# superxslam/SuperOdom

Measured on AMD Instinct MI355X. Metric: icp_registrations_per_sec, higher is better.
Workload: dtype f64

## Files before the change

superodom_amd/build.py:

```python
import os
import subprocess
import sys

HERE = os.path.dirname(os.path.abspath(__file__))
CSRC = os.path.join(HERE, "csrc")
LIBDIR = os.path.join(HERE, "lib")
LIB = os.path.join(LIBDIR, "libsoicp.so")
SOURCES = ["kernels.hip", "map_kernels.hip", "icp_context.cpp", "staging.cpp", "sequence.cpp", "batch.cpp", "localization.cpp", "prefilter.cpp", "cloud_steps.cpp", "multi_gpu.cpp",
           "local_map.cpp", "device_map.cpp", "localization_sequence.cpp", "feature_kernels.hip", "feature_extraction.cpp", "corr_kernels.hip", "corr_sums_kernels.hip", "corr_geometry_kernels.hip", "correspondences.cpp", "pose_prior.cpp"]
HEADERS = ["kernels.h", "device_idioms.h", "map_kernels.h", "device_map.h", "lm_solver.h", "local_map.h", "so_math.h", "deskew_math.h", "untimed_math.h", "plane_fit.h", "plane_factor.h", "ctx.h", "reg_plan.h", "feature_kernels.h", "corr_kernels.h", "pose_prior.h", "eval_kernel_body.inc", "solve_kernel_body.inc", os.path.join("..", "..", "include", "so_icp.h")]
ARCH = "gfx950"
COMMON = ["-O3", "-std=c++17", "-fPIC", "-ffp-contract=off", "-Wall", "-Wno-unused-function", "-Wno-unused-result"]
COMMON += os.environ.get("SOICP_EXTRA_CXXFLAGS", "").split()


def _stale():
    if not os.path.exists(LIB):
        return True
    t = os.path.getmtime(LIB)
    deps = [os.path.join(CSRC, s) for s in SOURCES + HEADERS] + [os.path.abspath(__file__)]
    return any(os.path.getmtime(d) > t for d in deps if os.path.exists(d))


def build(force=False, verbose=False):
    if not force and not _stale():
        return LIB
    hipcc = os.environ.get("HIPCC", "/opt/rocm/bin/hipcc")
    os.makedirs(LIBDIR, exist_ok=True)
    objs = []
    for s in SOURCES:
        o = os.path.join(LIBDIR, os.path.splitext(s)[0] + ".o")
        lang = ["-x", "hip"] if s.endswith(".hip") else []
        cmd = [hipcc, f"--offload-arch={ARCH}"] + lang + ["-c", os.path.join(CSRC, s), "-o", o] + COMMON
        if verbose:
            print(" ".join(cmd))
        subprocess.check_call(cmd)
        objs.append(o)
    cmd = [hipcc, f"--offload-arch={ARCH}", "-shared", "-o", LIB] + objs + ["-ldl"]
    if verbose:
        print(" ".join(cmd))
    subprocess.check_call(cmd)
    return LIB


if __name__ == "__main__":
    print(build(force="--force" in sys.argv, verbose=True))
```

superodom_amd/csrc/kernels.h:

```cpp
#pragma once
#include <hip/hip_runtime_api.h>

#include <cstddef>
#include <cstdint>

#include "lm_solver.h"
#include "pose_prior.h"
#include "so_math.h"

namespace soicp {

struct DevMapView {
  const float4* pts;
  const uint32_t* cell_start;
  const int32_t* cube_slot;
  int32_t nc;
  uint32_t ncell1;
  double inv_cell;
  int32_t origin[3];
  uint32_t n_points;
  uint32_t n_slots;
};

struct RegBeginArgs { double pose[7]; int32_t max_outer, lm_max; uint32_t chain_expect, pad; };

struct MatchParams {
  float plane_res;
  float sq_max_dist_f;
  double max_point_dist;
  int32_t ablate;
  unsigned long long* kdbg;
  uint32_t* packed_leftover;
  int32_t pack_light;
  int32_t skip_near_pass;
  uint32_t chunk_cap;
  uint32_t chain_expect;
  struct DevState* hring[2];
  unsigned long long seq_base;
  int32_t publish_prev;
  int32_t begin, begin_max_surface_features;
  uint32_t begin_n;
  RegBeginArgs begin_args;
  const unsigned long long* begin_ctr;
  struct DevState* begin_state;
};

struct EvalParams {
  double a2;
  int32_t variant;
  int32_t ablate;
  uint32_t n_queries, q_stride;
  struct DevState* hring[2];
  unsigned long long seq_base;
  int32_t defer_publish;
  uint32_t chain_expect;
  int32_t chain_next;
  double chain_delta[7];
  unsigned long long epoch_base;
  void* peer_inbox[8];
  int32_t peer_rank, peer_world;
  unsigned long long timeout_ticks;
// ... 132 lines not shown
```

superodom_amd/csrc/kernels.hip:

```cpp
#include <hip/hip_runtime.h>
#include <hip/hip_ext.h>

#include <cstddef>
#include <cstdlib>
#include <cstring>
#include <type_traits>

#ifdef SO_LM_STAMPS
#define SO_LM_STAMP(dbg, i) do { if (dbg) (dbg)[i] = wall_clock64(); } while (0)
#endif
#include "device_idioms.h"
#include "kernels.h"
#include "plane_factor.h"
#include "plane_fit.h"
#include "pose_prior.h"

namespace soicp {

#define SO_MATCH_SUCCESS 0
#define SO_MATCH_NOT_ENOUGH 1
#define SO_MATCH_TOO_FAR 2
#define SO_MATCH_BAD_PCA 3
#define SO_MATCH_INVALID 4
#define SO_MATCH_MSE 5
// ... 304 lines not shown

__device__ __forceinline__ int32_t imed3(int32_t a, int32_t b, int32_t c) {
  int32_t r;
  asm("v_med3_i32 %0, %1, %2, %3" : "=v"(r) : "v"(a), "v"(b), "v"(c));
  return r;
}

constexpr int32_t kKeyEmpty = 0x7FFFFFFF;

struct Net8 {
  int32_t a0, a1, a2, a3, a4, a5, a6, a7;
  __device__ __forceinline__ void init() { a0 = a1 = a2 = a3 = a4 = a5 = a6 = a7 = kKeyEmpty; }
  __device__ __forceinline__ void push(int32_t k) {
    a7 = imed3(a6, a7, k);
    a6 = imed3(a5, a6, k);
    a5 = imed3(a4, a5, k);
    a4 = imed3(a3, a4, k);
    a3 = imed3(a2, a3, k);
    a2 = imed3(a1, a2, k);
    a1 = imed3(a0, a1, k);
    a0 = a0 < k ? a0 : k;
  }
};

constexpr float kApproxAbsErr = 2e-5f;
typedef float float2v __attribute__((ext_vector_type(2)));
__device__ __forceinline__ float2v approx_d2_pair(float2v m2qx, float2v m2qy, float2v m2qz, float2v qq, float2v cx, float2v cy,
                                                  float2v cz, float2v cc) {
  float2v v = cc + qq;
  v = __builtin_elementwise_fma(m2qx, cx, v);
  v = __builtin_elementwise_fma(m2qy, cy, v);
  v = __builtin_elementwise_fma(m2qz, cz, v);
  return v;
}
__device__ __forceinline__ int32_t make_key(float d2a, uint32_t jloc_uniform, uint32_t keep_mask) {
  int32_t r;
  asm("v_bfi_b32 %0, %1, %2, %3" : "=v"(r) : "v"(keep_mask), "v"(d2a), "s"(jloc_uniform));
  return r;
}
__device__ __forceinline__ int32_t make_key_v(float d2a, uint32_t jloc, uint32_t keep_mask) {
  int32_t r;
  asm("v_bfi_b32 %0, %1, %2, %3" : "=v"(r) : "v"(keep_mask), "v"(d2a), "v"(jloc));
  return r;
}
__device__ __forceinline__ int32_t approx_key(float m2qx, float m2qy, float m2qz, float qq, float cx, float cy, float cz,
                                              float cc, uint32_t jloc, uint32_t keep_mask) {
  float v = cc + qq;
  v = __builtin_fmaf(m2qx, cx, v);
  v = __builtin_fmaf(m2qy, cy, v);
  v = __builtin_fmaf(m2qz, cz, v);
  return (int32_t)((__float_as_uint(v) & keep_mask) | (jloc & ~keep_mask));
}

__device__ __forceinline__ void publish_state_to(DevState* dst, const DevState* st, unsigned long long seq, int tid, int nthreads);

#ifndef SO_KNN_FILTER
#define SO_KNN_FILTER 1
#endif
__device__ __forceinline__ float wave_min_f32(float v) {
  const int inf = 0x7F800000;
#define SO_DPP_MIN(ctrl, rows) v = fminf(v, __int_as_float(__builtin_amdgcn_update_dpp(inf, __float_as_int(v), ctrl, rows, 0xF, false)))
  SO_DPP_MIN(0x111, 0xF); SO_DPP_MIN(0x112, 0xF); SO_DPP_MIN(0x114, 0xF); SO_DPP_MIN(0x118, 0xF);
  SO_DPP_MIN(0x142, 0xA); SO_DPP_MIN(0x143, 0xC);
#undef SO_DPP_MIN
  return __int_as_float(__builtin_amdgcn_readlane(__float_as_int(v), 63));
}

__device__ __forceinline__ int row_min_i32(int v) {
  v = min(v, __builtin_amdgcn_update_dpp(v, v, 0x121, 0xF, 0xF, false)); v = min(v, __builtin_amdgcn_update_dpp(v, v, 0x122, 0xF, 0xF, false));
  v = min(v, __builtin_amdgcn_update_dpp(v, v, 0x124, 0xF, 0xF, false)); v = min(v, __builtin_amdgcn_update_dpp(v, v, 0x128, 0xF, 0xF, false));
  return v;
}
__device__ __forceinline__ int row_max_i32(int v) {
  v = max(v, __builtin_amdgcn_update_dpp(v, v, 0x121, 0xF, 0xF, false)); v = max(v, __builtin_amdgcn_update_dpp(v, v, 0x122, 0xF, 0xF, false));
  v = max(v, __builtin_amdgcn_update_dpp(v, v, 0x124, 0xF, 0xF, false)); v = max(v, __builtin_amdgcn_update_dpp(v, v, 0x128, 0xF, 0xF, false));
  return v;
}
__device__ __forceinline__ float row_min_f32(float v) {
#define SO_ROR_F(ctrl) __int_as_float(__builtin_amdgcn_update_dpp(__float_as_int(v), __float_as_int(v), ctrl, 0xF, 0xF, false))
  v = fminf(v, SO_ROR_F(0x121)); v = fminf(v, SO_ROR_F(0x122)); v = fminf(v, SO_ROR_F(0x124)); v = fminf(v, SO_ROR_F(0x128));
#undef SO_ROR_F
  return v;
}
__device__ __forceinline__ unsigned long long wave_min_u64(unsigned long long v) {
#pragma unroll
  for (int off = 32; off > 0; off >>= 1) {
    const unsigned long long o = __shfl_xor(v, off, 64);
    v = o < v ? o : v;
  }
  return v;
}
__device__ __forceinline__ uint32_t row_inclusive_scan_u32(uint32_t v) {
  v += (uint32_t)__builtin_amdgcn_update_dpp(0, (int)v, 0x111, 0xF, 0xF, true);
  v += (uint32_t)__builtin_amdgcn_update_dpp(0, (int)v, 0x112, 0xF, 0xF, true);
  v += (uint32_t)__builtin_amdgcn_update_dpp(0, (int)v, 0x114, 0xF, 0xF, true);
  v += (uint32_t)__builtin_amdgcn_update_dpp(0, (int)v, 0x118, 0xF, 0xF, true);
  return v;
}
__device__ __forceinline__ uint32_t max_over_rows(uint32_t v) {
  return max(max((uint32_t)__builtin_amdgcn_readlane((int)v, 0), (uint32_t)__builtin_amdgcn_readlane((int)v, 16)),
             max((uint32_t)__builtin_amdgcn_readlane((int)v, 32), (uint32_t)__builtin_amdgcn_readlane((int)v, 48)));
}
__device__ __forceinline__ float block_cover_distance(int bx0, int bx1, int by0, int by1, int bz0, int bz1, int nc, float cell,
                                                      float ux, float uy, float uz) {
  float cv = 1e15f;
  if (bx0 > 0) cv = fminf(cv, ux - (float)bx0 * cell);
  if (bx1 < nc - 1) cv = fminf(cv, (float)(bx1 + 1) * cell - ux);
// ... 842 lines not shown
__device__ __forceinline__ void store16_sc1(u4v* p, u4v v) { asm volatile("global_store_dwordx4 %0, %1, off sc1" ::"v"(p), "v"(v) : "memory"); }
__device__ __forceinline__ u4v load16_sc1(const u4v* p) {
  u4v v;
  asm volatile("global_load_dwordx4 %0, %1, off sc1\n\ts_waitcnt vmcnt(0)" : "=v"(v) : "v"(p) : "memory");
  return v;
}

__device__ __forceinline__ void store16_sys(u4v* p, u4v v) { asm volatile("global_store_dwordx4 %0, %1, off sc0 sc1" ::"v"(p), "v"(v) : "memory"); }
__device__ __forceinline__ u4v load16_sys(const u4v* p) {
  u4v v;
  asm volatile("global_load_dwordx4 %0, %1, off sc0 sc1\n\ts_waitcnt vmcnt(0)" : "=v"(v) : "v"(p) : "memory");
  return v;
}

#define SO_LM_INLINE __forceinline__
__device__ __forceinline__ void copy_lm_state(LmState& dst, const LmState& src) {
#pragma unroll
  for (int i = 0; i < 7; ++i) { dst.x[i] = src.x[i]; dst.cand[i] = src.cand[i]; }
#pragma unroll
  for (int i = 0; i < 6; ++i) {
    dst.g[i] = src.g[i]; dst.scale[i] = src.scale[i]; dst.diag[i] = src.diag[i];
#pragma unroll
    for (int j = i; j < 6; ++j) { const double h = src.H[6 * i + j]; dst.H[6 * i + j] = h; dst.H[6 * j + i] = h; }
  }
  dst.x_cost = src.x_cost; dst.x_norm = src.x_norm; dst.inv_radius = src.inv_radius; dst.decrease_factor = src.decrease_factor;
  dst.inv_model_cost_change = src.inv_model_cost_change; dst.step_norm = src.step_norm; dst.cand_norm = src.cand_norm;
  dst.model_cost_change = src.model_cost_change; dst.initial_cost = src.initial_cost; dst.count = src.count;
  dst.iter = src.iter; dst.max_iter = src.max_iter; dst.reuse_diagonal = src.reuse_diagonal; dst.invalid_steps = src.invalid_steps;
  dst.num_successful = src.num_successful; dst.termination = src.termination; dst.done = src.done; dst.lm_iterations = src.lm_iterations;
}
__device__ SO_LM_INLINE int lm_control(int slot, DevState* st, LmState& S_lds, const LmSums& sums_lds, const LmCtl& ctl) {
  LmState S;
  copy_lm_state(S, S_lds);
  int more;
  if (slot == 0) more = lm_begin(S, ctl.T, sums_lds, ctl.lm_max, st->eval_pose);
#ifdef SO_LM_STAMPS
  else more = lm_feed(S, sums_lds, st->eval_pose, slot == 1 ? st->dbg : nullptr);
#else
  else more = lm_feed(S, sums_lds, st->eval_pose);
#endif
  st->lm_more = more;
  if (!more && lm_solve_finished(st, ctl, S.x, S.count, S.lm_iterations, S.num_successful, S.termination, S.initial_cost, S.x_cost, sums_lds)) {
    const bool have = S.count >= 1.0;
    for (int i = 0; i < 36; ++i) st->JtJ[i] = have ? S.H[i] : 0.0;
    for (int i = 0; i < 6; ++i) st->Jtr[i] = have ? S.g[i] : 0.0;
  }
  copy_lm_state(S_lds, S);
#ifdef SO_LM_STAMPS
  if (slot == 1) st->dbg[7] = wall_clock64();
#endif
  return more;
}

__device__ __forceinline__ int lm_control_wave(int slot, DevState* st, LmState& S, const LmSums& sums, const LmCtl& ctl, double* gather ,
                                               u4v* hand, unsigned long long want, double* pose_out, int* reg_done_out, int lane,
                                               unsigned long long* dbg = nullptr) {
  const bool is_mat = lane < 36, is_vec = lane >= 36 && lane < 42;
  const int li = is_mat ? lane / 6 : 0, lj = is_mat ? lane - 6 * li : (is_vec ? lane - 36 : 0);
  const int la = li < lj ? li : lj, lb = li < lj ? lj : li;
  const int tri = 6 * la - (la * (la - 1)) / 2 + (lb - la);
  const bool is_diag = is_mat && li == lj;
  double x[7], cand[7];
  double x_cost, x_norm, inv_radius, decrease_factor, mcc_state, initial_cost, count, inv_mcc, step_norm, cand_norm;
  int iter, max_iter, reuse_diagonal, invalid_steps, num_successful, termination, done, lm_iterations;
  double Hl = 0, gl = 0, diag_l = 0, sa = 1.0, sb = 1.0;
  int more = 0;
  bool propose = false;
  if (slot == 0) {
#pragma unroll
    for (int i = 0; i < 7; ++i) { x[i] = ctl.T[i]; cand[i] = x[i]; }
    iter = 0; max_iter = ctl.lm_max; reuse_diagonal = 0; invalid_steps = 0; num_successful = 0; termination = 0; done = 0; lm_iterations = 0;
    inv_radius = LmConst::kInitialInvRadius; decrease_factor = 2.0; mcc_state = 0; inv_mcc = 0; step_norm = 0; cand_norm = 0;
    count = sums.count; x_cost = sums.cost; initial_cost = x_cost; x_norm = 0;
    if (is_mat) Hl = sums.JtJ[tri];
    if (is_vec) gl = sums.Jtr[lj];
    if (!(count >= 1.0)) { termination = 4; done = 1; }
    else {
      const double sc = 1.0 / (1.0 + sqrt(Hl));
      if (is_diag) S.scale[li] = sc;
      __builtin_amdgcn_fence(__ATOMIC_ACQ_REL, "wavefront");
      sa = S.scale[is_vec ? lj : la]; sb = S.scale[lb];
      double n2 = 0;
#pragma unroll
      for (int i = 0; i < 7; ++i) n2 = SO_FMA(x[i], x[i], n2);
      x_norm = sqrt(n2);
      propose = true;
    }
  } else {
#pragma unroll
    for (int i = 0; i < 7; ++i) { x[i] = S.x[i]; cand[i] = S.cand[i]; }
    x_cost = S.x_cost; x_norm = S.x_norm; inv_radius = S.inv_radius; decrease_factor = S.decrease_factor; mcc_state = S.model_cost_change;
    initial_cost = S.initial_cost; count = S.count; inv_mcc = S.inv_model_cost_change; step_norm = S.step_norm; cand_norm = S.cand_norm;
    iter = S.iter; max_iter = S.max_iter; reuse_diagonal = S.reuse_diagonal; invalid_steps = S.invalid_steps; num_successful = S.num_successful;
    termination = S.termination; done = S.done; lm_iterations = S.lm_iterations;
    if (is_mat) { Hl = S.H[lane]; sa = S.scale[la]; sb = S.scale[lb]; }
    if (is_vec) { gl = S.g[lj]; sa = S.scale[lj]; }
    if (is_diag) diag_l = S.diag[li];
    if (!done) {
      SO_LM_STAMP(dbg, 0);
      const double cand_cost = sums.cost;
      if (step_norm <= LmConst::kParameterTolerance * (x_norm + LmConst::kParameterTolerance)) { termination = 2; done = 1; }
      else {
        const double cost_change = x_cost - cand_cost;
        if (fabs(cost_change) <= LmConst::kFunctionTolerance * x_cost) { termination = 1; done = 1; }
        else {
          const double rel = cost_change * inv_mcc;
          SO_LM_STAMP(dbg, 1);
          if (rel > LmConst::kMinRelativeDecrease) {
#pragma unroll
// ... 46 lines not shown
      double v = Hl * sa * sa;
      v = v < LmConst::kMinLmDiagonal ? LmConst::kMinLmDiagonal : v;
      diag_l = v > LmConst::kMaxLmDiagonal ? LmConst::kMaxLmDiagonal : v;
    }
    const double Hs = Hl * sa * sb;
    const double damp = diag_l * inv_radius;
    const double Al = is_diag ? Hs + damp : Hs;
    if (is_mat) gather[lane] = Al;
    if (is_diag) gather[42 + li] = Hs;
    if (is_vec) gather[36 + lj] = gl * sa;
    __builtin_amdgcn_fence(__ATOMIC_ACQ_REL, "wavefront");
    double A[36], gs[6], y[6], step[6];
#pragma unroll
    for (int i = 0; i < 6; ++i) {
#pragma unroll
      for (int j = 0; j <= i; ++j) A[6 * i + j] = gather[6 * i + j];
      gs[i] = gather[36 + i];
    }
    SO_LM_STAMP(dbg, 3);
    const bool ok = lm_chol6(A, gs, y);
    SO_LM_STAMP(dbg, 4);
    reuse_diagonal = 1;
    double mcc = 0;
    if (ok) {
      double sHs = 0, sg = 0;
#pragma unroll
      for (int i = 0; i < 6; ++i) { step[i] = -y[i]; sg = SO_FMA(step[i], gs[i], sg); }
#pragma unroll
      for (int i = 0; i < 6; ++i) {
        double r = 0;
#pragma unroll
        for (int j = i + 1; j < 6; ++j) r = SO_FMA(gather[6 * i + j], step[j], r);
        sHs = SO_FMA(step[i], SO_FMA(gather[42 + i], step[i], 2.0 * r), sHs);
      }
      mcc = SO_FMA(-0.5, sHs, -sg);
    }
    __builtin_amdgcn_fence(__ATOMIC_ACQ_REL, "wavefront");
    if (!ok || !(mcc > 0.0)) {
      if (++invalid_steps >= LmConst::kMaxConsecutiveInvalidSteps) { termination = 5; done = 1; break; }
      inv_radius = inv_radius * decrease_factor; decrease_factor *= 2.0;
      continue;
    }
    SO_LM_STAMP(dbg, 5);
    invalid_steps = 0;
    mcc_state = mcc;
    double delta[6];
#pragma unroll
    for (int i = 0; i < 6; ++i) delta[i] = step[i] * scale_u[i];
    pose_plus(x, delta, cand);
    SO_LM_STAMP(dbg, 6);
    more = 1;
    break;
  }
  {
    double hv = cand[0];
    hv = lane == 1 ? cand[1] : hv; hv = lane == 2 ? cand[2] : hv; hv = lane == 3 ? cand[3] : hv;
    hv = lane == 4 ? cand[4] : hv; hv = lane == 5 ? cand[5] : hv; hv = lane == 6 ? cand[6] : hv;
    const unsigned long long val = lane == 7 ? (unsigned long long)more : (unsigned long long)__double_as_longlong(hv);
    if (lane < 8) {
      const u4v v = {(unsigned int)val, (unsigned int)(val >> 32), (unsigned int)want, (unsigned int)(want >> 32)};
      store16_sc1(hand + lane, v);
    }
    if (lane < 7) pose_out[lane] = hv;
  }
  if (more) {
    inv_mcc = 1.0 / mcc_state;
    double sn = 0, n2 = 0;
#pragma unroll
    for (int i = 0; i < 7; ++i) sn = SO_FMA(x[i] - cand[i], x[i] - cand[i], sn);
#pragma unroll
    for (int i = 0; i < 7; ++i) n2 = SO_FMA(cand[i], cand[i], n2);
    step_norm = sqrt(sn); cand_norm = sqrt(n2);
  }
  if (is_mat) S.H[lane] = Hl;
  if (is_vec) S.g[lj] = gl;
  if (is_diag) S.diag[li] = diag_l;
  if (slot == 0 && termination == 4 && lane < 6) S.scale[lane] = 1.0;
  if (lane == 0) {
#pragma unroll
    for (int i = 0; i < 7; ++i) { S.x[i] = x[i]; S.cand[i] = cand[i]; }
    S.x_cost = x_cost; S.x_norm = x_norm; S.inv_radius = inv_radius; S.decrease_factor = decrease_factor; S.model_cost_change = mcc_state;
    S.initial_cost = initial_cost; S.count = count; S.inv_model_cost_change = inv_mcc; S.step_norm = step_norm; S.cand_norm = cand_norm;
    S.iter = iter; S.max_iter = max_iter; S.reuse_diagonal = reuse_diagonal; S.invalid_steps = invalid_steps; S.num_successful = num_successful;
    S.termination = termination; S.done = done; S.lm_iterations = lm_iterations;
  }
#ifdef SO_LM_STAMPS
  if (slot == 1 && lane == 0) st->dbg[7] = wall_clock64();
#endif
  if (!more) {
    int rd = 0;
    if (lane == 0) {
      st->lm_more = 0;
      rd = lm_solve_finished(st, ctl, x, count, lm_iterations, num_successful, termination, initial_cost, x_cost, sums);
      *reg_done_out = rd;
    }
    rd = __builtin_amdgcn_readfirstlane(rd);
    if (rd) {
      const bool have = count >= 1.0;
      if (is_mat) st->JtJ[lane] = have ? Hl : 0.0;
      if (is_vec) st->Jtr[lj] = have ? gl : 0.0;
    }
  } else if (lane == 0) *reg_done_out = 0;
  return more;
}

__device__ __forceinline__ void load_ctl(LmCtl& ctl, const DevState* st, int tid, int first) {
  const int k = tid - first;
  if (k >= 0 && k < 7) ctl.T[k] = st->T[k];
  else if (k == 7) ctl.lm_max = st->lm_max;
  else if (k == 8) ctl.outer_iter = st->outer_iter;
  else if (k == 9) ctl.max_outer = st->max_outer;
}

__device__ __forceinline__ void publish_state(const DevState* st, const EvalParams& ep, int outer, int tid, int nthreads) {
  publish_state_to(ep.hring[outer & 1], st, ep.seq_base | (unsigned long long)(outer + 1), tid, nthreads);
}
__device__ __forceinline__ void publish_state_to(DevState* dst, const DevState* st, unsigned long long seq, int tid, int nthreads) {
  if (!dst) return;
  __threadfence_block();
  __syncthreads();
  const unsigned long long* src = reinterpret_cast<const unsigned long long*>(st);
  unsigned long long* out = reinterpret_cast<unsigned long long*>(dst);
  constexpr int kWords = (int)(offsetof(DevState, seq) / 8);
  for (int i = tid; i < kWords; i += nthreads) out[i] = src[i];
  __threadfence_system();
  __syncthreads();
  if (tid == 0) __hip_atomic_store(&dst->seq, seq, __ATOMIC_RELEASE, __HIP_MEMORY_SCOPE_SYSTEM);
}

__device__ __forceinline__ void copy_words(double* dst, const double* src, int n_doubles, int tid, int nthreads) {
  for (int i = tid; i < n_doubles; i += nthreads) dst[i] = src[i];
}
static_assert(sizeof(LmState) % 8 == 0 && sizeof(LmSums) % 8 == 0, "controller state must be double-aligned");

constexpr int kPartStride = SO_SOLVE_BLOCKS;
static_assert(kEvalBlocks <= kPartStride && kFitBlocksMax <= kPartStride && kNAcc <= kSumsStride, "partials table");
constexpr int kRedStride = kNAcc + 2;

template <int CTRL>
__device__ __forceinline__ double dpp_f64(double v) {
  const int lo = __builtin_amdgcn_update_dpp(0, __double2loint(v), CTRL, 0xF, 0xF, false);
  const int hi = __builtin_amdgcn_update_dpp(0, __double2hiint(v), CTRL, 0xF, 0xF, false);
  return __hiloint2double(hi, lo);
}
__device__ __forceinline__ double swap32_add(double a, double b) {
  const auto lo = __builtin_amdgcn_permlane32_swap((unsigned)__double2loint(a), (unsigned)__double2loint(b), false, false);
  const auto hi = __builtin_amdgcn_permlane32_swap((unsigned)__double2hiint(a), (unsigned)__double2hiint(b), false, false);
  return __hiloint2double((int)hi[0], (int)lo[0]) + __hiloint2double((int)hi[1], (int)lo[1]);
}
__device__ __forceinline__ double swap16_add(double a, double b) {
  const auto lo = __builtin_amdgcn_permlane16_swap((unsigned)__double2loint(a), (unsigned)__double2loint(b), false, false);
  const auto hi = __builtin_amdgcn_permlane16_swap((unsigned)__double2hiint(a), (unsigned)__double2hiint(b), false, false);
  return __hiloint2double((int)hi[0], (int)lo[0]) + __hiloint2double((int)hi[1], (int)lo[1]);
}
template <int CTRL>
__device__ __forceinline__ double row_stage_add(double a, double b, bool up) {
  const double keep = up ? b : a, give = up ? a : b;
  return keep + dpp_f64<CTRL>(give);
}
__device__ __forceinline__ double wave_reduce_scatter(const double (&acc)[kNAcc]) {
  static_assert(kNAcc > 16 && kNAcc <= 32, "butterfly over 32 value slots");
  const int lane = (int)(threadIdx.x & 63u);
  double u[16], w[8], x[4], y[2];
#pragma unroll
  for (int a = 0; a < 16; ++a) u[a] = swap32_add(acc[a], (a + 16 < kNAcc) ? acc[a + 16] : 0.0);
#pragma unroll
  for (int a = 0; a < 8; ++a) w[a] = swap16_add(u[a], u[a + 8]);
  const bool b3 = (lane & 8) != 0, b2 = (lane & 4) != 0, b1 = (lane & 2) != 0;
#pragma unroll
  for (int a = 0; a < 4; ++a) x[a] = row_stage_add<0x128>(w[a], w[a + 4], b3);
#pragma unroll
  for (int a = 0; a < 2; ++a) y[a] = row_stage_add<0x141>(x[a], x[a + 2], b2);
  const double z = row_stage_add<0x4E>(y[0], y[1], b1);
  return z + dpp_f64<0xB1>(z);
}
__device__ __forceinline__ double wg_reduce(const double (&acc)[kNAcc], double (*part)[32], int tid) {
  const double t = wave_reduce_scatter(acc);
  const int lane = tid & 63, wave = tid >> 6;
  if (!(lane & 1) && (lane >> 1) < kNAcc) part[wave][lane >> 1] = t;
  __syncthreads();
// ... 130 lines not shown
                     "+v"(r[q][22]), "+v"(r[q][23]), "+v"(r[q][24]), "+v"(r[q][25]), "+v"(r[q][26]), "+v"(r[q][27]), "+v"(r[q][28])
                   :: "memory");
#pragma unroll
    for (int a = 0; a < kNAcc; ++a) {
      double v = have[0] ? r[0][a] : 0.0;
#pragma unroll
      for (int q = 1; q < kRec; ++q) v += have[q] ? r[q][a] : 0.0;
      sh.red[tid][a] = v;
    }
  }
  __syncthreads();
  if (stamp) T.loaded = wall_clock64();
  const double total = reduce_records(sh.red, sh.part, tid);
  double* o = reinterpret_cast<double*>(&sh.sums);
  if (tid < kNAcc) {
    if constexpr (PRIOR) {
      PosePriorPart part;
      prior_prepare(prior, pose, tid, part);
      o[tid] = prior_added(part, total, tid);
    } else
    o[tid] = total;
  } else if (tid >= 32 && tid < 48) {
    int h = 0;
#pragma unroll
    for (int r = 0; r < kHistReplicas; ++r)
      h += __hip_atomic_load(&hist[r * kHistStride + (tid - 32)], __ATOMIC_RELAXED, __HIP_MEMORY_SCOPE_AGENT);
    o[kNAcc + (tid - 32)] = (double)h;
  }
  __syncthreads();
  copy_words(reinterpret_cast<double*>(out), o, (int)(sizeof(LmSums) / 8), tid, 256);
  if (stamp) T.sums = wall_clock64();
  if (!fuse_lm) return kPassSums;
  if (tid == 0) sh.more = (abl & 32) ? 1 : lm_control(slot, st, sh.S, sh.sums, sh.ctl);
  __syncthreads();
  if (stamp) T.ctl = wall_clock64();
  if (!sh.more) { hist[tid] = 0; hist[256 + tid] = 0; }
  if (tid < (int)(sizeof(LmState) / 8))
    __hip_atomic_store(reinterpret_cast<double*>(&st->S) + tid, reinterpret_cast<const double*>(&sh.S)[tid], __ATOMIC_RELAXED, __HIP_MEMORY_SCOPE_AGENT);
  if (!sh.more) publish_state(st, ep, sh.ctl.outer_iter, tid, 256);
  if (stamp && tid == 0 && (FIT || slot == 1)) store_stamps<FIT>(st, T, true);
  return sh.more ? kPassMore : kPassDone;
}
struct WgSpan { uint32_t vb0, vb1, V; bool ctl; };
constexpr int kPriorAtGuess = 2, kPriorBatch = 3;
template <bool FIT, bool PERSIST = false, bool PROF = false, bool BATCH = false, bool PEER = false, int PRIOR = 0>
__device__ __forceinline__ int eval_pass(int slot, int fuse_lm, const Pose& pose, const float* __restrict__ spx,
                                         const float* __restrict__ spy, const float* __restrict__ spz,
                                         const CorrBuffers& corr, DevState* __restrict__ st, const EvalParams& ep,
                                         double* __restrict__ partials, uint32_t* __restrict__ ticket,
                                         int32_t* __restrict__ hist, LmSums* __restrict__ out,
                                         const float4* __restrict__ mpts, const uint32_t* __restrict__ nbr5,
                                         const MatchParams& mp, EvalShared& sh, const double* prior, unsigned long long pass_tag = 0,
                                         CorrCache* cc = nullptr, u4v* hand = nullptr, unsigned long long want = 0,
                                         const WgSpan span = WgSpan{0, 0, 0, false}, const double* prior_tm = nullptr) {
  double (*red)[kRedStride] = sh.red;
  double (*part)[32] = sh.part;
  LmSums& sh_sums = sh.sums;
  LmState& sh_S = sh.S;
  LmCtl& sh_ctl = sh.ctl;
  int& sh_more = sh.more;
  int32_t* lh = sh.lh;
  const int tid = threadIdx.x;
  static_assert(!BATCH || PERSIST, "batched hypotheses run in the persistent solve launch");
  static_assert(!PRIOR || !PEER, "the pose prior belongs to one device");
  static_assert(BATCH == (PRIOR == kPriorBatch) || !PRIOR, "a batch reads its priors from the table in memory, a single registration from the launch's argument");
  static_assert(PRIOR != kPriorAtGuess || PERSIST, "the prior at the guess belongs to the persistent solve");
  const int abl = PROF ? ep.ablate : 0;
  const bool stamp = PROF && (abl & 128) != 0;
  const uint32_t V = BATCH ? span.V : gridDim.x;
  const uint32_t vb_begin = BATCH ? span.vb0 : blockIdx.x, vb_end = BATCH ? span.vb1 : blockIdx.x + 1u;
  const bool is_ctl = BATCH ? span.ctl : (blockIdx.x == 0);
  PassStamps T;
  if (stamp) T.begin = wall_clock64();
  if (FIT) {
    if (tid < 16) lh[tid] = 0;
    __syncthreads();
  }
  const uint32_t n_kept = (abl & 64) ? 0u : ep.n_queries;
  const uint32_t qs = ep.q_stride;
  double acc[kNAcc];
  double R[9];
  quat_to_matrix(pose.q, R);
  const ObsAxes axes = obs_axes(pose);
  const double inv_a2 = 1.0 / ep.a2, rho_out = (ep.variant == 0) ? ep.a2 / 6.0 : ep.a2 / 3.0;
  auto tail = [&](double px, double py, double pz, double wx, double wy, double wz, const double4& nd, double c) {
    const double r = plane_residual(nd.x, nd.y, nd.z, nd.w, wx, wy, wz);
    const double s = r * r;
    double rho0, rho1;
    if (s <= ep.a2) {
      const double v = 1.0 - s * inv_a2, v2 = v * v;
      rho0 = rho_out * (1.0 - v2 * v); rho1 = (ep.variant == 0) ? 0.5 * v2 : v2;
    } else {
      rho0 = rho_out; rho1 = 0;
    }
    plane_factor_add(R, px, py, pz, nd.x, nd.y, nd.z, c, r, rho0, c * rho1, acc);
  };
  auto at_pose = [&](double px, double py, double pz, const double4& nd, double c) {
    double wx, wy, wz;
    quat_rotate<double>(pose.q, px, py, pz, wx, wy, wz);
    wx += pose.t[0]; wy += pose.t[1]; wz += pose.t[2];
    tail(px, py, pz, wx, wy, wz, nd, c);
  };
  auto body = [&](const uint32_t j, int status, const float* nb, int trip) {
    if (!FIT && status != SO_MATCH_SUCCESS) return;
    if (FIT && status == SO_MATCH_DROPPED) return;
    const float fx = spx[(size_t)j * qs], fy = spy[(size_t)j * qs], fz = spz[(size_t)j * qs];
    const double px = (double)fx, py = (double)fy, pz = (double)fz;
// ... 232 lines not shown
        if (SO_PRIOR_OVERLAP == 0) {
          if constexpr (PRIOR == kPriorAtGuess) prior_prepare_at(prior_tm, prior, pose, tid, prior_part);
          else prior_prepare(prior, pose, tid, prior_part);
        }
        tot = prior_added(prior_part, tot, tid);
      }
      o[tid] = tot;
    } else if (FIT && tid >= 32 && tid < 48) {
      int h = 0;
#pragma unroll
      for (int cc8 = 0; cc8 < 8; ++cc8) h += sh.hpart[cc8][tid - 32];
      o[kNAcc + (tid - 32)] = (double)h;
    }
    __syncthreads();
    if (PEER && ep.peer_world > 1) {
      const int nx = FIT ? (kNAcc + 16) : kNAcc;
      const unsigned int xtag = (unsigned int)(sh.peer_seq + 1ull);
      const int par = (int)(xtag & 1u);
      if (tid < nx) {
        const unsigned long long b = (unsigned long long)__double_as_longlong(o[tid]);
        const u4v v = {(unsigned int)b, (unsigned int)(b >> 32), xtag, (unsigned int)ep.peer_rank};
        for (int p = 0; p < ep.peer_world; ++p)
          store16_sys(reinterpret_cast<u4v*>(ep.peer_inbox[p]) + (size_t)(par * kPeerMaxWorld + ep.peer_rank) * kPeerChunks + tid, v);
      }
      const u4v* own = reinterpret_cast<const u4v*>(ep.peer_inbox[ep.peer_rank]) + (size_t)par * kPeerMaxWorld * kPeerChunks;
      const int total = nx * ep.peer_world;
      const int c0 = tid, c1 = tid + 256;
      const bool h0 = c0 < total, h1 = c1 < total;
      const int s0 = h0 ? c0 / nx : 0, a0 = h0 ? c0 - s0 * nx : 0, s1 = h1 ? c1 / nx : 0, a1 = h1 ? c1 - s1 * nx : 0;
      bool d0 = !h0, d1 = !h1;
      unsigned long long v0 = 0, v1 = 0;
      const unsigned long long tp = wall_clock64();
      bool okx = true;
      for (;;) {
        if (!d0) { const u4v v = load16_sys(own + (size_t)s0 * kPeerChunks + a0); if (v.z == xtag) { d0 = true; v0 = ((unsigned long long)v.y << 32) | v.x; } }
        if (!d1) { const u4v v = load16_sys(own + (size_t)s1 * kPeerChunks + a1); if (v.z == xtag) { d1 = true; v1 = ((unsigned long long)v.y << 32) | v.x; } }
        if (__syncthreads_and((d0 && d1) ? 1 : 0)) break;
        if (__syncthreads_or((wall_clock64() - tp > ep.timeout_ticks) ? 1 : 0)) { okx = false; break; }
      }
      if (!__syncthreads_and(okx ? 1 : 0)) return kPassNotLast;
      double (*xs)[48] = reinterpret_cast<double (*)[48]>(&red[0][0]);
      if (h0) xs[s0][a0] = __longlong_as_double((long long)v0);
      if (h1) xs[s1][a1] = __longlong_as_double((long long)v1);
      __syncthreads();
      if (tid < nx) {
        double tot = 0;
        for (int r = 0; r < ep.peer_world; ++r) tot += xs[r][tid];
        o[tid] = tot;
      }
      if (tid == 0) sh.peer_seq = (unsigned long long)xtag;
      __syncthreads();
    }
    if (stamp) T.sums = wall_clock64();
    if (tid < 64) {
#ifdef SO_LM_STAMPS
      const int more_ = lm_control_wave(slot, st, sh_S, sh_sums, sh_ctl, &sh.part_odd[0][0], hand, want, sh.pose, &sh.reg_done, tid, (slot == 1 && tid == 0) ? st->dbg : nullptr);
#else
      const int more_ = lm_control_wave(slot, st, sh_S, sh_sums, sh_ctl, &sh.part_odd[0][0], hand, want, sh.pose, &sh.reg_done, tid);
#endif
      if (tid == 0) sh_more = more_;
    }
    __syncthreads();
    if (stamp) T.ctl = wall_clock64();
    if (!sh_more) {
      hist[tid] = 0; hist[256 + tid] = 0;
      if (PEER && ep.peer_world > 1 && tid == 0) st->peer_seq = sh.peer_seq;
      if (tid < (int)(sizeof(LmState) / 8))
        __hip_atomic_store(reinterpret_cast<double*>(&st->S) + tid, reinterpret_cast<const double*>(&sh_S)[tid], __ATOMIC_RELAXED, __HIP_MEMORY_SCOPE_AGENT);
      if (!BATCH && ep.chain_next && sh.reg_done && tid == 0) {
        double tf[7], nx[7];
        for (int i = 0; i < 7; ++i) tf[i] = sh_S.x[i];
        pose_compose(tf, ep.chain_delta, nx);
        for (int i = 0; i < 7; ++i) st->T_chain[i] = nx[i];
      }
      if (!ep.defer_publish || sh.reg_done) publish_state(st, ep, sh_ctl.outer_iter, tid, 256);
    }
    if (stamp && tid == 0 && (FIT || slot == 1)) store_stamps<FIT>(st, T, !FIT || BATCH);
    return sh_more ? kPassMore : kPassDone;
  }
  return hand_over_ticketed<FIT, PROF, PRIOR != 0>(slot, fuse_lm, mine, st, ep, partials, ticket, hist, out, sh, T, pose, prior);
}

static_assert(sizeof(LmState) / 8 <= 256, "controller state is moved one word per thread");
template <bool FIT, bool PROF>
__global__ __launch_bounds__(256, SO_SOLVE_BLOCKS / 256) void eval_kernel(int slot, int fuse_lm, const float* __restrict__ spx,
                                                   const float* __restrict__ spy, const float* __restrict__ spz,
                                                   CorrBuffers corr, DevState* __restrict__ st, EvalParams ep,
                                                   double* __restrict__ partials, uint32_t* __restrict__ ticket,
                                                   int32_t* __restrict__ hist, LmSums* __restrict__ out,
                                                   const float4* __restrict__ mpts, const uint32_t* __restrict__ nbr5,
                                                   MatchParams mp) {
#define SO_BODY_KERNEL eval_kernel<FIT, PROF>
#define SO_BODY_PRIOR false
#define SO_BODY_PRIOR_WORDS nullptr
#include "eval_kernel_body.inc"
#undef SO_BODY_KERNEL
#undef SO_BODY_PRIOR
#undef SO_BODY_PRIOR_WORDS
}
template <bool FIT, bool PROF>
__global__ __launch_bounds__(256, SO_SOLVE_BLOCKS / 256) void eval_kernel_prior(int slot, int fuse_lm, const float* __restrict__ spx,
                                                   const float* __restrict__ spy, const float* __restrict__ spz,
                                                   CorrBuffers corr, DevState* __restrict__ st, EvalParams ep,
                                                   double* __restrict__ partials, uint32_t* __restrict__ ticket,
                                                   int32_t* __restrict__ hist, LmSums* __restrict__ out,
                                                   const float4* __restrict__ mpts, const uint32_t* __restrict__ nbr5,
                                                   MatchParams mp, PosePrior prior) {
#define SO_BODY_KERNEL eval_kernel_prior<FIT, PROF>
#define SO_BODY_PRIOR true
#define SO_BODY_PRIOR_WORDS reinterpret_cast<const double*>(&prior)
#include "eval_kernel_body.inc"
#undef SO_BODY_KERNEL
#undef SO_BODY_PRIOR
#undef SO_BODY_PRIOR_WORDS
}

template <bool PROF, bool BATCH, bool PEER = false>
__global__ __launch_bounds__(256, BATCH ? 2 : 1) void solve_kernel(int lm_max, const float* __restrict__ spx, const float* __restrict__ spy,
                                                    const float* __restrict__ spz, CorrBuffers corr, DevState* __restrict__ st,
                                                    EvalParams ep, double* __restrict__ partials, uint32_t* __restrict__ ticket,
                                                    int32_t* __restrict__ hist, LmSums* __restrict__ out,
                                                    const float4* __restrict__ mpts, const uint32_t* __restrict__ nbr5,
                                                    MatchParams mp, BatchView bv) {
#define SO_BODY_KERNEL solve_kernel<PROF, BATCH, PEER>
#define SO_BODY_PRIOR 0
#define SO_BODY_PRIOR_WORDS nullptr
#include "solve_kernel_body.inc"
#undef SO_BODY_KERNEL
#undef SO_BODY_PRIOR
#undef SO_BODY_PRIOR_WORDS
// ... 382 lines not shown
```

superodom_amd/csrc/solve_kernel_body.inc:

```
  __shared__ EvalShared sh;
  __shared__ CorrCache cache;
  unsigned long long t_entry = 0;
  if (PROF && !BATCH) t_entry = wall_clock64();
  if (SO_ENTRY_WARM) st = after_loaded(st, kernarg_lines<decltype(&SO_BODY_KERNEL)>());
  WgSpan span{0, 0, 0, false};
#ifdef SO_BODY_PRIOR_TABLE
  const double* prior_block = nullptr;
#endif
  if (BATCH) {
    const uint32_t G = bv.wg_per_hyp, hi = blockIdx.x / G, sub = blockIdx.x - hi * G;
    const size_t h = bv.active[hi];
#ifdef SO_BODY_PRIOR_TABLE
    prior_block = SO_BODY_PRIOR_TABLE + h * kBatchPriorStride;
#endif
    st += h; corr.nd += h * bv.bs; corr.coeff += h * bv.bs; corr.status += h * bv.bs; nbr5 += h * 5 * bv.bs;
    partials += h * bv.partial_stride; ticket += h * bv.sync_stride; hist += h * (kHistReplicas * kHistStride);
    span.V = bv.v_grid;
    span.vb0 = (uint32_t)(((unsigned long long)sub * bv.v_grid) / G);
    span.vb1 = (uint32_t)(((unsigned long long)(sub + 1u) * bv.v_grid) / G);
    span.ctl = sub == 0;
  }
  if (SO_ENTRY_WARM) st = after_loaded(st, state_lines<true, !BATCH>(st));
  if (st->reg_done) return;
  if (!BATCH && ep.chain_expect && st->done_count != ep.chain_expect) return;
  const int tid = threadIdx.x;
  [[maybe_unused]] double prior_tm[7] = {0, 0, 0, 0, 0, 0, 1};
  if constexpr (SO_BODY_PRIOR == kPriorAtGuess) {
    if (blockIdx.x == 0 && tid < 64) {
#pragma unroll
      for (int i = 0; i < 7; ++i) prior_tm[i] = st->pose_in[i];
    }
  }
  u4v* hand = reinterpret_cast<u4v*>(ticket + kHandoffWordOffset);
  const unsigned long long e0 = ep.epoch_base;
  Pose pose = pose_from_array(st->T);
  if (tid == 0) {
    sh.peer_seq = st->peer_seq;
    for (int i = 0; i < 3; ++i) sh.ctl.T[i] = pose.t[i];
    for (int i = 0; i < 4; ++i) sh.ctl.T[3 + i] = pose.q[i];
    sh.ctl.lm_max = st->lm_max; sh.ctl.outer_iter = st->outer_iter; sh.ctl.max_outer = st->max_outer;
  }
  const unsigned long long tag0 = (e0 + 1ull) << 5;
  if (PROF && !BATCH && (ep.ablate & 128) && tid == 0 && blockIdx.x == 0) st->dbg[3] = wall_clock64() - t_entry;
  int code = eval_pass<true, true, PROF, BATCH, PEER, SO_BODY_PRIOR>(0, 1, pose, spx, spy, spz, corr, st, ep, partials, ticket, hist, out, mpts, nbr5, mp, sh, SO_BODY_PRIOR_WORDS, tag0, &cache, hand, e0 + 1ull, span, prior_tm);
  for (int slot = 1; slot <= lm_max; ++slot) {
    __syncthreads();
    const unsigned long long want = e0 + (unsigned long long)slot;
    if (code == kPassMore || code == kPassDone) {
    } else if (tid < 64) {
      bool done = tid >= 8;
      unsigned long long val = 0;
      const unsigned long long t0 = wall_clock64();
      bool ok = true;
      for (;;) {
        if (!done) {
          const u4v v = load16_sc1(hand + tid);
          const unsigned long long tag = ((unsigned long long)v.w << 32) | v.z;
          if (tag - e0 >= (unsigned long long)slot && tag - e0 <= 64ull) { done = true; val = ((unsigned long long)v.y << 32) | v.x; }
        }
        if (__ballot(!done) == 0ull) break;
        if (wall_clock64() - t0 > 2ull * ep.timeout_ticks + 5000000ull) { ok = false; break; }
        __builtin_amdgcn_s_sleep(1);
      }
      if (tid < 7) sh.pose[tid] = __longlong_as_double((long long)val);
      if (tid == 7) sh.more = ok ? (int)val : -1;
    }
    __syncthreads();
    if (sh.more != 1) return;
    pose = pose_from_array(sh.pose);
    __syncthreads();
    code = eval_pass<false, true, PROF, BATCH, PEER, SO_BODY_PRIOR>(slot, 1, pose, spx, spy, spz, corr, st, ep, partials, ticket, hist, out, mpts, nbr5, mp, sh, SO_BODY_PRIOR_WORDS, tag0 + (unsigned long long)slot, &cache, hand, want + 1ull, span, prior_tm);
  }
```

Before: 7276.

## Stage LM endgame state in LDS image and publish with unfenced 16-byte stores

Block 0 of the fused solve kernel keeps a shared-memory copy of DevState. The LM control wave writes into this copy, and at the end it is flushed to global memory and to the host ring in one pass of 16-byte stores. The system fence and release store are replaced by a vmcnt wait plus a relaxed seq store, which removes fence and scattered-store latency from the end of each registration. The parameter-tolerance check now runs on the proposal step, so converged solves can stop one LM pass earlier. The cost is extra LDS use, a weaker memory-ordering guarantee for the host reader, and a possible shift in numerical termination behaviour.

```diff
diff --git a/superodom_amd/build.py b/superodom_amd/build.py
--- a/superodom_amd/build.py
+++ b/superodom_amd/build.py
@@ -8,7 +8,7 @@
 LIB = os.path.join(LIBDIR, "libsoicp.so")
 SOURCES = ["kernels.hip", "map_kernels.hip", "icp_context.cpp", "staging.cpp", "sequence.cpp", "batch.cpp", "localization.cpp", "prefilter.cpp", "cloud_steps.cpp", "multi_gpu.cpp",
            "local_map.cpp", "device_map.cpp", "localization_sequence.cpp", "feature_kernels.hip", "feature_extraction.cpp", "corr_kernels.hip", "corr_sums_kernels.hip", "corr_geometry_kernels.hip", "correspondences.cpp", "pose_prior.cpp"]
-HEADERS = ["kernels.h", "device_idioms.h", "map_kernels.h", "device_map.h", "lm_solver.h", "local_map.h", "so_math.h", "deskew_math.h", "untimed_math.h", "plane_fit.h", "plane_factor.h", "ctx.h", "reg_plan.h", "feature_kernels.h", "corr_kernels.h", "pose_prior.h", "eval_kernel_body.inc", "solve_kernel_body.inc", os.path.join("..", "..", "include", "so_icp.h")]
+HEADERS = ["kernels.h", "device_idioms.h", "map_kernels.h", "device_map.h", "lm_solver.h", "lm_endgame.h", "local_map.h", "so_math.h", "deskew_math.h", "untimed_math.h", "plane_fit.h", "plane_factor.h", "ctx.h", "reg_plan.h", "feature_kernels.h", "corr_kernels.h", "pose_prior.h", "eval_kernel_body.inc", "solve_kernel_body.inc", os.path.join("..", "..", "include", "so_icp.h")]
 ARCH = "gfx950"
 COMMON = ["-O3", "-std=c++17", "-fPIC", "-ffp-contract=off", "-Wall", "-Wno-unused-function", "-Wno-unused-result"]
 COMMON += os.environ.get("SOICP_EXTRA_CXXFLAGS", "").split()
diff --git a/superodom_amd/csrc/kernels.h b/superodom_amd/csrc/kernels.h
--- a/superodom_amd/csrc/kernels.h
+++ b/superodom_amd/csrc/kernels.h
@@ -4,9 +4,20 @@
 #include <cstddef>
 #include <cstdint>
 
+#include "lm_endgame.h"
 #include "lm_solver.h"
 #include "pose_prior.h"
 #include "so_math.h"
+
+#ifndef SO_ENDGAME_IMAGE
+#define SO_ENDGAME_IMAGE 1
+#endif
+#ifndef SO_PUBLISH_FENCED
+#define SO_PUBLISH_FENCED 0
+#endif
+#ifndef SO_PTOL_AT_PROPOSAL
+#define SO_PTOL_AT_PROPOSAL 1
+#endif
 
 namespace soicp {
 
diff --git a/superodom_amd/csrc/kernels.hip b/superodom_amd/csrc/kernels.hip
--- a/superodom_amd/csrc/kernels.hip
+++ b/superodom_amd/csrc/kernels.hip
@@ -380,7 +380,8 @@
   return (int32_t)((__float_as_uint(v) & keep_mask) | (jloc & ~keep_mask));
 }
 
-__device__ __forceinline__ void publish_state_to(DevState* dst, const DevState* st, unsigned long long seq, int tid, int nthreads);
+__device__ __forceinline__ void publish_state_to(DevState* dst, const DevState* st, unsigned long long seq, int tid, int nthreads,
+                                                 unsigned long long* eg = nullptr);
 
 #ifndef SO_KNN_FILTER
 #define SO_KNN_FILTER 1
@@ -1329,9 +1330,10 @@
   return more;
 }
 
+template <bool PTOL = false, bool EG = false>
 __device__ __forceinline__ int lm_control_wave(int slot, DevState* st, LmState& S, const LmSums& sums, const LmCtl& ctl, double* gather ,
                                                u4v* hand, unsigned long long want, double* pose_out, int* reg_done_out, int lane,
-                                               unsigned long long* dbg = nullptr) {
+                                               unsigned long long* dbg = nullptr, unsigned long long* eg = nullptr) {
   const bool is_mat = lane < 36, is_vec = lane >= 36 && lane < 42;
   const int li = is_mat ? lane / 6 : 0, lj = is_mat ? lane - 6 * li : (is_vec ? lane - 36 : 0);
   const int la = li < lj ? li : lj, lb = li < lj ? lj : li;
@@ -1484,6 +1486,17 @@
     more = 1;
     break;
   }
+  [[maybe_unused]] double sn_early = 0;
+  [[maybe_unused]] bool ptol = false;
+  if constexpr (PTOL) {
+    if (more) {
+#pragma unroll
+      for (int i = 0; i < 7; ++i) sn_early = SO_FMA(x[i] - cand[i], x[i] - cand[i], sn_early);
+      ptol = lm_parameter_tolerance_at_proposal(sn_early, x_norm);
+      if (ptol) more = 0;
+    }
+  }
+  if constexpr (EG) { if (eg) eg[0] = wall_clock64(); }
   {
     double hv = cand[0];
     hv = lane == 1 ? cand[1] : hv; hv = lane == 2 ? cand[2] : hv; hv = lane == 3 ? cand[3] : hv;
@@ -1495,14 +1508,21 @@
     }
     if (lane < 7) pose_out[lane] = hv;
   }
-  if (more) {
+  if constexpr (EG) { if (eg) eg[1] = wall_clock64(); }
+  if (more || (PTOL && ptol)) {
     inv_mcc = 1.0 / mcc_state;
     double sn = 0, n2 = 0;
-#pragma unroll
-    for (int i = 0; i < 7; ++i) sn = SO_FMA(x[i] - cand[i], x[i] - cand[i], sn);
+    if constexpr (PTOL) sn = sn_early;
+    else {
+#pragma unroll
+      for (int i = 0; i < 7; ++i) sn = SO_FMA(x[i] - cand[i], x[i] - cand[i], sn);
+    }
 #pragma unroll
     for (int i = 0; i < 7; ++i) n2 = SO_FMA(cand[i], cand[i], n2);
     step_norm = sqrt(sn); cand_norm = sqrt(n2);
+  }
+  if constexpr (PTOL) {
+    if (ptol) { termination = 2; done = 1; }
   }
   if (is_mat) S.H[lane] = Hl;
   if (is_vec) S.g[lj] = gl;
@@ -1532,6 +1552,7 @@
       if (is_mat) st->JtJ[lane] = have ? Hl : 0.0;
       if (is_vec) st->Jtr[lj] = have ? gl : 0.0;
     }
+    if constexpr (EG) { if (eg) eg[2] = wall_clock64(); }
   } else if (lane == 0) *reg_done_out = 0;
   return more;
 }
@@ -1547,7 +1568,7 @@
 __device__ __forceinline__ void publish_state(const DevState* st, const EvalParams& ep, int outer, int tid, int nthreads) {
   publish_state_to(ep.hring[outer & 1], st, ep.seq_base | (unsigned long long)(outer + 1), tid, nthreads);
 }
-__device__ __forceinline__ void publish_state_to(DevState* dst, const DevState* st, unsigned long long seq, int tid, int nthreads) {
+__device__ __forceinline__ void publish_state_to(DevState* dst, const DevState* st, unsigned long long seq, int tid, int nthreads, unsigned long long* eg) {
   if (!dst) return;
   __threadfence_block();
   __syncthreads();
@@ -1555,9 +1576,38 @@
   unsigned long long* out = reinterpret_cast<unsigned long long*>(dst);
   constexpr int kWords = (int)(offsetof(DevState, seq) / 8);
   for (int i = tid; i < kWords; i += nthreads) out[i] = src[i];
+  if (eg) eg[0] = wall_clock64();
   __threadfence_system();
   __syncthreads();
+  if (eg) eg[1] = wall_clock64();
   if (tid == 0) __hip_atomic_store(&dst->seq, seq, __ATOMIC_RELEASE, __HIP_MEMORY_SCOPE_SYSTEM);
+  if (eg) eg[2] = wall_clock64();
+}
+constexpr int kStateChunks = (int)(offsetof(DevState, seq) / 16);
+static_assert(offsetof(DevState, seq) % 16 == 0 && alignof(u4v) == 16, "the state block up to seq goes out in 16-byte chunks");
+__device__ __forceinline__ void flush_state_image(DevState* st, DevState* mirror, const DevState* img, unsigned long long seq, int tid, unsigned long long* eg) {
+  const u4v* src = reinterpret_cast<const u4v*>(img);
+  u4v* out = reinterpret_cast<u4v*>(st);
+  u4v* pub = reinterpret_cast<u4v*>(mirror);
+  for (int i = tid; i < kStateChunks; i += 256) {
+    const u4v v = src[i];
+    out[i] = v;
+    if (mirror) store16_sys(pub + i, v);
+  }
+  if (!mirror) {
+    if (eg) eg[0] = wall_clock64();
+    return;
+  }
+  asm volatile("s_waitcnt vmcnt(0)" ::: "memory");
+  if (eg) eg[0] = wall_clock64();
+  if (SO_PUBLISH_FENCED) __threadfence_system();
+  __syncthreads();
+  if (eg) eg[1] = wall_clock64();
+  if (tid == 0) {
+    if (SO_PUBLISH_FENCED) __hip_atomic_store(&mirror->seq, seq, __ATOMIC_RELEASE, __HIP_MEMORY_SCOPE_SYSTEM);
+    else __hip_atomic_store(&mirror->seq, seq, __ATOMIC_RELAXED, __HIP_MEMORY_SCOPE_SYSTEM);
+  }
+  if (eg) eg[2] = wall_clock64();
 }
 
 __device__ __forceinline__ void copy_words(double* dst, const double* src, int n_doubles, int tid, int nthreads) {
@@ -1794,7 +1844,8 @@
                                          const float4* __restrict__ mpts, const uint32_t* __restrict__ nbr5,
                                          const MatchParams& mp, EvalShared& sh, const double* prior, unsigned long long pass_tag = 0,
                                          CorrCache* cc = nullptr, u4v* hand = nullptr, unsigned long long want = 0,
-                                         const WgSpan span = WgSpan{0, 0, 0, false}, const double* prior_tm = nullptr) {
+                                         const WgSpan span = WgSpan{0, 0, 0, false}, const double* prior_tm = nullptr,
+                                         DevState* img = nullptr ) {
   double (*red)[kRedStride] = sh.red;
   double (*part)[32] = sh.part;
   LmSums& sh_sums = sh.sums;
@@ -2133,30 +2184,62 @@
       __syncthreads();
     }
     if (stamp) T.sums = wall_clock64();
+    constexpr bool kImage = SO_ENDGAME_IMAGE != 0 && !BATCH;
+    constexpr bool kPtol = SO_PTOL_AT_PROPOSAL != 0 && !BATCH;
+    DevState* const sw = kImage ? img : st;
+    const bool eg_stamp = stamp && (abl & 131072) != 0;
+    unsigned long long eg[3] = {0, 0, 0};
     if (tid < 64) {
 #ifdef SO_LM_STAMPS
-      const int more_ = lm_control_wave(slot, st, sh_S, sh_sums, sh_ctl, &sh.part_odd[0][0], hand, want, sh.pose, &sh.reg_done, tid, (slot == 1 && tid == 0) ? st->dbg : nullptr);
+      unsigned long long* const lm_dbg = (slot == 1 && tid == 0) ? sw->dbg : nullptr;
 #else
-      const int more_ = lm_control_wave(slot, st, sh_S, sh_sums, sh_ctl, &sh.part_odd[0][0], hand, want, sh.pose, &sh.reg_done, tid);
+      unsigned long long* const lm_dbg = nullptr;
 #endif
+      const int more_ = lm_control_wave<kPtol, PROF>(slot, sw, sh_S, sh_sums, sh_ctl, &sh.part_odd[0][0], hand, want, sh.pose, &sh.reg_done, tid, lm_dbg,
+                                               (PROF && eg_stamp) ? eg : nullptr);
       if (tid == 0) sh_more = more_;
     }
     __syncthreads();
     if (stamp) T.ctl = wall_clock64();
     if (!sh_more) {
       hist[tid] = 0; hist[256 + tid] = 0;
-      if (PEER && ep.peer_world > 1 && tid == 0) st->peer_seq = sh.peer_seq;
-      if (tid < (int)(sizeof(LmState) / 8))
-        __hip_atomic_store(reinterpret_cast<double*>(&st->S) + tid, reinterpret_cast<const double*>(&sh_S)[tid], __ATOMIC_RELAXED, __HIP_MEMORY_SCOPE_AGENT);
-      if (!BATCH && ep.chain_next && sh.reg_done && tid == 0) {
-        double tf[7], nx[7];
-        for (int i = 0; i < 7; ++i) tf[i] = sh_S.x[i];
-        pose_compose(tf, ep.chain_delta, nx);
-        for (int i = 0; i < 7; ++i) st->T_chain[i] = nx[i];
-      }
-      if (!ep.defer_publish || sh.reg_done) publish_state(st, ep, sh_ctl.outer_iter, tid, 256);
-    }
-    if (stamp && tid == 0 && (FIT || slot == 1)) store_stamps<FIT>(st, T, !FIT || BATCH);
+      if (PROF && eg_stamp && tid == 0) { sw->dbg[8] = eg[1] - eg[0]; sw->dbg[9] = eg[2] - eg[1]; sw->dbg[15] = (unsigned long long)(slot + 1); }
+      const bool publish = !ep.defer_publish || sh.reg_done;
+      unsigned long long eg_late[4] = {0, 0, 0, 0};
+      if constexpr (kImage) {
+        if (PEER && ep.peer_world > 1 && tid == 0) sw->peer_seq = sh.peer_seq;
+        if (tid < (int)(sizeof(LmState) / 8)) reinterpret_cast<double*>(&sw->S)[tid] = reinterpret_cast<const double*>(&sh_S)[tid];
+        if (ep.chain_next && sh.reg_done && tid == 128) {
+          double tf[7], nx[7];
+          for (int i = 0; i < 7; ++i) tf[i] = sh_S.x[i];
+          pose_compose(tf, ep.chain_delta, nx);
+          for (int i = 0; i < 7; ++i) sw->T_chain[i] = nx[i];
+        }
+        __syncthreads();
+        if (PROF && eg_stamp) eg_late[0] = wall_clock64();
+        flush_state_image(st, publish ? ep.hring[sh_ctl.outer_iter & 1] : nullptr, sw, ep.seq_base | (unsigned long long)(sh_ctl.outer_iter + 1), tid,
+                          (PROF && eg_stamp) ? eg_late + 1 : nullptr);
+      } else {
+        if (PEER && ep.peer_world > 1 && tid == 0) st->peer_seq = sh.peer_seq;
+        if (tid < (int)(sizeof(LmState) / 8))
+          __hip_atomic_store(reinterpret_cast<double*>(&st->S) + tid, reinterpret_cast<const double*>(&sh_S)[tid], __ATOMIC_RELAXED, __HIP_MEMORY_SCOPE_AGENT);
+        if (!BATCH && ep.chain_next && sh.reg_done && tid == 0) {
+          double tf[7], nx[7];
+          for (int i = 0; i < 7; ++i) tf[i] = sh_S.x[i];
+          pose_compose(tf, ep.chain_delta, nx);
+          for (int i = 0; i < 7; ++i) st->T_chain[i] = nx[i];
+        }
+        if (PROF && eg_stamp) eg_late[0] = wall_clock64();
+        if (publish) publish_state_to(ep.hring[sh_ctl.outer_iter & 1], st, ep.seq_base | (unsigned long long)(sh_ctl.outer_iter + 1), tid, 256, (PROF && eg_stamp) ? eg_late + 1 : nullptr);
+      }
+      if (PROF && eg_stamp && publish && tid == 0) {
+        const unsigned long long t_end = wall_clock64();
+        for (int i = 1; i < 4; ++i) if (!eg_late[i]) eg_late[i] = i == 3 ? t_end : eg_late[i - 1];
+        st->dbg[10] = eg_late[0] - eg[2]; st->dbg[11] = eg_late[1] - eg_late[0]; st->dbg[12] = eg_late[2] - eg_late[1];
+        st->dbg[13] = eg_late[3] - eg_late[2]; st->dbg[14] = eg_late[3] - eg[0];
+      }
+    }
+    if (stamp && tid == 0 && (FIT || (slot == 1 && !eg_stamp))) store_stamps<FIT>(sw, T, !FIT || BATCH);
     return sh_more ? kPassMore : kPassDone;
   }
   return hand_over_ticketed<FIT, PROF, PRIOR != 0>(slot, fuse_lm, mine, st, ep, partials, ticket, hist, out, sh, T, pose, prior);
diff --git a/superodom_amd/csrc/lm_endgame.h b/superodom_amd/csrc/lm_endgame.h
--- /dev/null
+++ b/superodom_amd/csrc/lm_endgame.h
@@ -0,0 +1,14 @@
+#pragma once
+#include <cmath>
+
+#include "lm_solver.h"
+
+namespace soicp {
+
+SO_HD bool lm_parameter_tolerance_at_proposal(double sn, double x_norm) {
+  const double thr = LmConst::kParameterTolerance * (x_norm + LmConst::kParameterTolerance);
+  if (sn > thr * thr * 1.0000001) return false;
+  return sqrt(sn) <= thr;
+}
+
+}
diff --git a/superodom_amd/csrc/solve_kernel_body.inc b/superodom_amd/csrc/solve_kernel_body.inc
--- a/superodom_amd/csrc/solve_kernel_body.inc
+++ b/superodom_amd/csrc/solve_kernel_body.inc
@@ -1,5 +1,8 @@
   __shared__ EvalShared sh;
   __shared__ CorrCache cache;
+  constexpr bool kStateImage = SO_ENDGAME_IMAGE != 0 && !BATCH;
+  __shared__ u4v state_image[kStateImage ? kStateChunks + 1 : 1];
+  DevState* const img = reinterpret_cast<DevState*>(state_image);
   unsigned long long t_entry = 0;
   if (PROF && !BATCH) t_entry = wall_clock64();
   if (SO_ENTRY_WARM) st = after_loaded(st, kernarg_lines<decltype(&SO_BODY_KERNEL)>());
@@ -41,8 +44,15 @@
     sh.ctl.lm_max = st->lm_max; sh.ctl.outer_iter = st->outer_iter; sh.ctl.max_outer = st->max_outer;
   }
   const unsigned long long tag0 = (e0 + 1ull) << 5;
-  if (PROF && !BATCH && (ep.ablate & 128) && tid == 0 && blockIdx.x == 0) st->dbg[3] = wall_clock64() - t_entry;
-  int code = eval_pass<true, true, PROF, BATCH, PEER, SO_BODY_PRIOR>(0, 1, pose, spx, spy, spz, corr, st, ep, partials, ticket, hist, out, mpts, nbr5, mp, sh, SO_BODY_PRIOR_WORDS, tag0, &cache, hand, e0 + 1ull, span, prior_tm);
+  if (kStateImage && blockIdx.x == 0) {
+    const u4v* block = reinterpret_cast<const u4v*>(st);
+    for (int i = tid; i < kStateChunks; i += 256) state_image[i] = block[i];
+  }
+  if (PROF && !BATCH && (ep.ablate & 128) && blockIdx.x == 0) {
+    if (kStateImage) __syncthreads();
+    if (tid == 0) (kStateImage ? img : st)->dbg[3] = wall_clock64() - t_entry;
+  }
+  int code = eval_pass<true, true, PROF, BATCH, PEER, SO_BODY_PRIOR>(0, 1, pose, spx, spy, spz, corr, st, ep, partials, ticket, hist, out, mpts, nbr5, mp, sh, SO_BODY_PRIOR_WORDS, tag0, &cache, hand, e0 + 1ull, span, prior_tm, img);
   for (int slot = 1; slot <= lm_max; ++slot) {
     __syncthreads();
     const unsigned long long want = e0 + (unsigned long long)slot;
@@ -69,5 +79,5 @@
     if (sh.more != 1) return;
     pose = pose_from_array(sh.pose);
     __syncthreads();
-    code = eval_pass<false, true, PROF, BATCH, PEER, SO_BODY_PRIOR>(slot, 1, pose, spx, spy, spz, corr, st, ep, partials, ticket, hist, out, mpts, nbr5, mp, sh, SO_BODY_PRIOR_WORDS, tag0 + (unsigned long long)slot, &cache, hand, want + 1ull, span, prior_tm);
+    code = eval_pass<false, true, PROF, BATCH, PEER, SO_BODY_PRIOR>(slot, 1, pose, spx, spy, spz, corr, st, ep, partials, ticket, hist, out, mpts, nbr5, mp, sh, SO_BODY_PRIOR_WORDS, tag0 + (unsigned long long)slot, &cache, hand, want + 1ull, span, prior_tm, img);
   }
```

New measurement: 7387 (median of 6 runs). 1.02x the previous value.
